# yuanzhi-zhu/DiffPIR

Measured on AMD Instinct MI355X. Metric: restored images/sec @100 NFE, 256x256, higher is better.
Workload: dtype f32 (GEMMs as 3 x f16 MFMA on hi/lo-split fp32 operands, fp32 accumulate; exact-fp32-MFMA mode in alt_precision); 1 GPU; configs[1]: ffhq topology 256x256 deblur (61x61 Gaussian PSF), 100 NFE, batch 16/GPU, device Philox noise, hipGraph=on; global_batch=16, nfe=100, collective=none

## Files before the change

### diffpir_amd/_lib.py

```python
from __future__ import annotations

import ctypes as C
import os

_HERE = os.path.dirname(os.path.abspath(__file__))
LIB_PATH = os.environ.get("DIFFPIR_LIB") or os.path.join(_HERE, "csrc", "libdiffpir_hip.so")
ABI_VERSION = 2



class UNetDesc(C.Structure):
    _fields_ = [("image_size", C.c_int32), ("in_channels", C.c_int32), ("model_channels", C.c_int32),
                ("out_channels", C.c_int32), ("num_res_blocks", C.c_int32), ("num_head_channels", C.c_int32),
                ("n_channel_mult", C.c_int32), ("channel_mult", C.c_float * 8),
                ("n_attention_ds", C.c_int32), ("attention_ds", C.c_int32 * 8), ("num_classes", C.c_int32)]


class Tensor(C.Structure):
    _fields_ = [("name", C.c_char_p), ("data", C.c_void_p), ("ndim", C.c_int32), ("shape", C.c_int64 * 4)]


class Step(C.Structure):
    _fields_ = [("t", C.c_int32), ("last", C.c_int32), ("c1", C.c_float), ("c2", C.c_float), ("tau", C.c_float),
                ("sa_t", C.c_float), ("s1m_t", C.c_float), ("sa_p", C.c_float),
# ... 9 lines not shown
                ("seed", C.c_uint64), ("image_offset", C.c_int64), ("use_graph", C.c_int32),
                ("skip_dead_final_eval", C.c_int32), ("generate_mode", C.c_int32), ("first_order", C.c_int32),
                ("noise_rp_dev", C.c_void_p), ("ddim_sample", C.c_int32)]


class InpaintRow(C.Structure):
    _fields_ = [("t", C.c_int32), ("last", C.c_int32), ("pos", C.c_int32), ("back", C.c_int32),
                ("c1", C.c_float), ("c2", C.c_float), ("tau", C.c_float), ("sa_t", C.c_float), ("s1m_t", C.c_float), ("sa_p", C.c_float),
                ("k1", C.c_float), ("q", C.c_float), ("es", C.c_float), ("k2", C.c_float),
                ("sae", C.c_float), ("sb", C.c_float), ("sa_n", C.c_float), ("s1m_n", C.c_float),
                ("mix_next", C.c_int32), ("reserved", C.c_int32)]


class DpsCoef(C.Structure):
    _fields_ = [("pc1", C.c_float), ("pc2", C.c_float), ("min_log", C.c_float), ("max_log", C.c_float), ("sa_prev", C.c_float), ("s1m_prev", C.c_float)]


class PSampleCoef(C.Structure):
    _fields_ = [("c1", C.c_float), ("c2", C.c_float), ("pc1", C.c_float), ("pc2", C.c_float), ("min_log", C.c_float), ("max_log", C.c_float),
                ("ddim", C.c_int32), ("sa_prev", C.c_float), ("s1m_prev", C.c_float)]


class DegradeDesc(C.Structure):
    _fields_ = [("task", C.c_int32), ("B", C.c_int32), ("H", C.c_int32), ("W", C.c_int32), ("sf", C.c_int32),
                ("kh", C.c_int32), ("kw", C.c_int32), ("noise_level_img", C.c_float), ("seed", C.c_uint64), ("image_offset", C.c_int64)]


class Conv3Desc(C.Structure):
    _fields_ = ([(n, C.c_int32) for n in ("B", "ca", "cb", "Cout", "H", "W", "mode", "res_mode", "scaled", "prologue", "route", "split",
                                          "defer", "Cout2")] +
                [(n, C.c_void_p) for n in ("xa", "xb", "w", "bias", "res", "prm", "gamma", "beta", "film", "gamma2", "beta2", "w2", "bias2",
                                           "out", "stat_out", "out2")] +
                [(n, C.c_int32) for n in ("stat_kind_out", "path_out", "ksplit_out", "reserved")])


PROF_CLASSES = 8
PROF_NAMES = ["conv3x3", "conv1x1", "groupnorm_stats", "attention", "fft_prox", "elementwise", "unet_forward", "loop_graph"]

SIGNATURES = {
    "dpir_version": (C.c_int, []),
    "dpir_device_count": (C.c_int, [C.POINTER(C.c_int)]),
    "dpir_create": (C.c_int, [C.c_int, C.POINTER(C.c_void_p)]),
    "dpir_destroy": (None, [C.c_void_p]),
    "dpir_last_error": (C.c_char_p, [C.c_void_p]),
    "dpir_sync": (C.c_int, [C.c_void_p]),
    "dpir_stream": (C.c_void_p, [C.c_void_p]),
    "dpir_malloc": (C.c_int, [C.c_void_p, C.c_size_t, C.POINTER(C.c_void_p)]),
    "dpir_free": (C.c_int, [C.c_void_p, C.c_void_p]),
    "dpir_h2d": (C.c_int, [C.c_void_p, C.c_void_p, C.c_void_p, C.c_size_t]),
    "dpir_d2h": (C.c_int, [C.c_void_p, C.c_void_p, C.c_void_p, C.c_size_t]),
    "dpir_d2d": (C.c_int, [C.c_void_p, C.c_void_p, C.c_void_p, C.c_size_t]),
    "dpir_load_unet": (C.c_int, [C.c_void_p, C.POINTER(UNetDesc), C.POINTER(Tensor), C.c_int]),
    "dpir_set_precision": (C.c_int, [C.c_void_p, C.c_int]),
    "dpir_unet_forward": (C.c_int, [C.c_void_p, C.c_void_p, C.c_void_p, C.c_void_p, C.c_void_p, C.c_int, C.c_int, C.c_int]),
    "dpir_model_fn_xstart": (C.c_int, [C.c_void_p, C.c_void_p, C.c_int, C.c_float, C.c_float, C.c_void_p, C.c_void_p,
                                       C.c_int, C.c_int, C.c_int]),
    "dpir_enable_grad": (C.c_int, [C.c_void_p, C.c_int]),
    "dpir_unet_vjp": (C.c_int, [C.c_void_p, C.c_void_p, C.c_void_p, C.c_void_p, C.c_void_p, C.c_void_p, C.c_void_p, C.c_int, C.c_int, C.c_int]),
    "dpir_run_dps_loop": (C.c_int, [C.c_void_p, C.POINTER(LoopDesc), C.POINTER(Step), C.POINTER(DpsCoef), C.c_int, C.c_int, C.c_float,
                                    C.c_void_p, C.c_void_p, C.c_float, C.c_void_p, C.c_void_p]),
    "dpir_p_sample": (C.c_int, [C.c_void_p, C.c_void_p, C.c_int, C.POINTER(PSampleCoef), C.c_void_p, C.c_void_p, C.c_void_p, C.c_void_p, C.c_int, C.c_int, C.c_int]),
    "dpir_eps_from_xstart": (C.c_int, [C.c_void_p, C.c_void_p, C.c_void_p, C.c_float, C.c_float, C.c_int, C.c_void_p, C.c_size_t]),
    "dpir_grad_and_value": (C.c_int, [C.c_void_p, C.c_int, C.c_void_p, C.c_void_p, C.c_int, C.c_void_p, C.c_void_p, C.c_int, C.c_int, C.c_int]),
    "dpir_blur_reflect": (C.c_int, [C.c_void_p, C.c_void_p, C.c_void_p, C.c_int, C.c_int, C.c_float, C.c_float, C.c_void_p, C.c_int, C.c_int, C.c_int]),
    "dpir_blur_reflect_adjoint": (C.c_int, [C.c_void_p, C.c_void_p, C.c_void_p, C.c_int, C.c_int, C.c_float, C.c_void_p, C.c_int, C.c_int, C.c_int]),
    "dpir_grad_and_value_blur": (C.c_int, [C.c_void_p, C.c_int, C.c_void_p, C.c_void_p, C.c_void_p, C.c_int, C.c_int, C.c_void_p, C.c_void_p,
# ... 41 lines not shown
}

_lib = None


class EngineLibraryError(RuntimeError):
    pass


DEBUG_LIB_PATH = os.path.join(_HERE, "csrc", "libdiffpir_dbg.so")
_dbg = None


def load_debug():
    global _dbg
    if _dbg is not None:
        return _dbg
    load()
    if not os.path.exists(DEBUG_LIB_PATH):
        raise EngineLibraryError(f"{DEBUG_LIB_PATH} not found: `make -C diffpir_amd/csrc` builds it next to the product library")
    d = C.CDLL(DEBUG_LIB_PATH)
    d.dpir_debug_conv_bench.argtypes = [C.c_void_p] + [C.c_int] * 10 + [C.POINTER(C.c_double)]
    d.dpir_debug_conv7_emit_supported.argtypes = [C.c_void_p] + [C.c_int] * 4 + [C.POINTER(C.c_int)]
    d.dpir_debug_victim.argtypes = [C.c_void_p, C.c_int, C.c_int, C.c_int, C.c_longlong, C.c_int, C.POINTER(C.c_ulonglong)]
    d.dpir_debug_victim_alu.argtypes = [C.c_void_p, C.c_int, C.c_int, C.c_int, C.c_int, C.POINTER(C.c_ulonglong)]
    for fn in (d.dpir_debug_victim_fft_pk, d.dpir_debug_victim_fft_nopk):
        fn.argtypes = [C.c_void_p, C.c_int, C.c_int, C.c_int, C.POINTER(C.c_ulonglong)]
    d.dpir_debug_conv7_check.argtypes = [C.c_void_p] + [C.c_int] * 10 + [C.POINTER(C.c_double), C.POINTER(C.c_double), C.POINTER(C.c_ulonglong),
                                                                        C.POINTER(C.c_float), C.POINTER(C.c_int)]
    d.dpir_debug_conv5_layer.argtypes = [C.c_void_p] + [C.c_int] * 7 + [C.c_void_p] * 7 + [C.POINTER(C.c_int)]
    d.dpir_debug_conv5_layer.restype = C.c_int
    d.dpir_debug_conv3_layer.argtypes = [C.c_void_p, C.POINTER(Conv3Desc)]
    d.dpir_debug_conv3_layer.restype = C.c_int
    for n in ("dpir_debug_conv_bench", "dpir_debug_victim", "dpir_debug_victim_alu", "dpir_debug_victim_fft_pk", "dpir_debug_victim_fft_nopk",
              "dpir_debug_conv7_check"):
        getattr(d, n).restype = C.c_int
    _dbg = d
    return d


def load():
    global _lib
    if _lib is not None:
        return _lib
    if not os.path.exists(LIB_PATH):
        raise EngineLibraryError(
            f"{LIB_PATH} not found: build it with `python -c 'import __graft_entry__ as g; g.build()'` "
            f"or `make -C diffpir_amd/csrc`.  There is no CPU fallback.")
    try:
        import torch
    except ImportError:
        pass
    try:
        lib = C.CDLL(LIB_PATH)
    except OSError as ex:
        raise EngineLibraryError(f"cannot load {LIB_PATH}: {ex}") from ex
    for name, (res, args) in SIGNATURES.items():
        try:
            fn = getattr(lib, name)
        except AttributeError as ex:
            raise EngineLibraryError(f"{LIB_PATH} does not export {name}") from ex
        fn.restype = res
        fn.argtypes = args
    if lib.dpir_version() != ABI_VERSION:
        raise EngineLibraryError("ABI version mismatch")
    _lib = lib
# ... 2 lines not shown
```

### diffpir_amd/csrc/dbg_conv.hip

```cpp
#include "engine.h"
#include "conv6_params.h"
#include "../../include/diffpir_debug.h"
#include <string.h>
#include <vector>
using namespace dpir;
static int fail(dpir_engine* e, const Status& s) {
    if (e) e->last_error = s.msg;
    return s.code;
}
#define API_TRY(e, expr)                          \
    do {                                          \
        Status _s = (expr);                       \
        if (!_s.ok()) return fail((e), _s);       \
    } while (0)
#define API_HIP(e, expr)                                                                  \
    do {                                                                                  \
        hipError_t _h = (expr);                                                           \
        if (_h != hipSuccess)                                                             \
            return fail((e), Status{DPIR_ERR_HIP, std::string(#expr) + ": " + hipGetErrorString(_h)}); \
    } while (0)

__global__ void dbg_bitdiff_kernel(const float* a, const float* b, size_t n, unsigned long long* out) {
    unsigned long long cnt = 0; unsigned mx = 0;
    for (size_t i = (size_t)blockIdx.x * blockDim.x + threadIdx.x; i < n; i += (size_t)gridDim.x * blockDim.x) {
        const float x = a[i], y = b[i];
        if (__builtin_bit_cast(unsigned, x) != __builtin_bit_cast(unsigned, y)) {
            ++cnt;
            const float d = fabsf(x - y);
            const unsigned u = d == d ? __builtin_bit_cast(unsigned, d) : 0x7fc00000u;
            mx = u > mx ? u : mx;
        }
    }
    if (cnt) { atomicAdd(&out[0], cnt); atomicMax(&out[1], (unsigned long long)mx); }
}
// ... 424 lines not shown
        ga.silu = true; ga.mode = 0; ga.B = B; ga.Hs = H; ga.Ws = W;
        ga.hi = s16b; ga.lo = x1 ? nullptr : s16b + plane2; ga.range_ctr = e->range_ctr;
        API_TRY(e, launch_gn_act_small(e->stream, ga));
        std::vector<uint16_t> w16b;
        const float w16b_scale = pack_weights_conv6(d->w2, Co2, Cn, w16b);
        void* wp2 = nullptr;
        API_TRY(e, e->ws.get("c3#w16b", w16b.size() * 2, &wp2));
        API_HIP(e, hipMemcpy(wp2, w16b.data(), w16b.size() * 2, hipMemcpyHostToDevice));
        Conv6Args c6;
        c6.x1 = x1; c6.xhi = s16b; c6.xlo = s16b + plane2; c6.w16 = wp2; c6.w16_scale = w16b_scale;
        c6.bias = dbias2; c6.out = dout2; c6.B = B; c6.Cin = Cn; c6.Cout = Co2; c6.H = H; c6.W = W;
        API_TRY(e, launch_conv6(e->stream, c6));
        API_HIP(e, hipStreamSynchronize(e->stream));
        API_HIP(e, hipMemcpy(d->out2, dout2, no2 * 4, hipMemcpyDeviceToHost));
    }
    API_HIP(e, hipStreamSynchronize(e->stream));
    API_HIP(e, hipMemcpy(d->out, dout, no * 4, hipMemcpyDeviceToHost));
    if (d->stat_out && (kind == 1 || kind == 2)) {
        if (kind == 1) {
            std::vector<float2> hs(nst);
            API_HIP(e, hipMemcpy(hs.data(), st, nst * 8, hipMemcpyDeviceToHost));
            for (size_t pl = 0; pl < (size_t)B * Cout; ++pl) {
                double s1 = 0.0, s2 = 0.0;
                for (int k = 0; k < slots; ++k) { s1 += (double)hs[pl * slots + k].x; s2 += (double)hs[pl * slots + k].y; }
                d->stat_out[2 * pl] = s1; d->stat_out[2 * pl + 1] = s2;
            }
        } else {
            API_HIP(e, hipMemcpy(d->stat_out, sp, (size_t)B * Cout * 16, hipMemcpyDeviceToHost));
        }
    }
    return DPIR_OK;
}

int dpir_debug_conv7_emit_supported(dpir_engine* e, int B, int Cout, int H, int W, int* capacity_out) {
    if (!e) return 0;
    (void)hipSetDevice(e->device);
    if (capacity_out) *capacity_out = conv7_emit_capacity();
    return conv7_emit_supported(B, Cout, H, W) ? 1 : 0;
}

}
```

### diffpir_amd/csrc/unet.hip

```cpp
#include "engine.h"
#include "conv6_params.h"
#include <unordered_map>
#include <cstdint>
#include <math.h>
#include <string.h>
#include <stdlib.h>

namespace dpir {

Status Workspace::get(const std::string& name, size_t bytes, void** out) {
    auto it = bufs.find(name);
    if (it != bufs.end() && it->second.bytes >= bytes) { *out = it->second.p; return Status{}; }
    if (frozen) return Status{DPIR_ERR_STATE, "workspace allocation of '" + name + "' during graph capture"};
    if (it != bufs.end()) { (void)hipFree(it->second.p); total -= it->second.bytes; bufs.erase(it); }
    void* p = nullptr;
    size_t rb = (bytes + 255) & ~(size_t)255;
    hipError_t err = hipMalloc(&p, rb);
    if (err != hipSuccess) return Status{DPIR_ERR_NOMEM, "hipMalloc(" + std::to_string(rb) + ") for '" + name + "' failed"};
    bufs[name] = DevBuf{p, rb};
    total += rb;
    ++generation;
    *out = p;
    return Status{};
}
void Workspace::release() {
    for (auto& kv : bufs) (void)hipFree(kv.second.p);
    bufs.clear();
    total = 0;
}

namespace {
struct WeightMap {
    std::map<std::string, const dpir_tensor*> m;
    Status find(const std::string& key, std::vector<int64_t> shape, const float** out) const {
// ... 288 lines not shown
            if (is_pending(res)) return invalid("gn_conv: residual is an unfinished convolution");
            const int C8 = 2 * ((C + 15) / 16);
            const size_t plane = (size_t)B * C8 * Ho * Wo * 16;
            char* s16 = nullptr;
            DPIR_TRY(ws.getT("act#s16", 2 * plane, &s16));
            GnActArgs ga;
            ga.src = CatSrc{in.a, in.ca, in.b, in.cb};
            ga.pend = pending;
            ga.gamma = g.gamma; ga.beta = g.beta;
            ga.film = film_off >= 0 ? film : nullptr; ga.film_stride = film_stride; ga.film_off = film_off < 0 ? 0 : film_off;
            ga.fstep = fstep; ga.frows = film_rows;
            ga.silu = true; ga.mode = mode; ga.B = B; ga.Hs = in.H; ga.Ws = in.W;
            ga.hi = s16; ga.lo = x1 ? nullptr : s16 + plane; ga.range_ctr = e->range_ctr;
            if (grad) {
                DPIR_TRY(ws.getT(tag + "#prm", (size_t)B * C, &ga.prm_out));
                DPIR_TRY(ws.getT(tag + "#gst", (size_t)B * 32, &ga.stats_out));
                if (prm_out) *prm_out = ga.prm_out;
                if (stats_out) *stats_out = ga.stats_out;
            }
            {
                ProfScope ps(&e->prof, PC_ELEM);
                DPIR_TRY(launch_gn_act_small(s, ga));
            }
            if (pending.partial) { fused.erase(pending.out); pending = PendingConv{}; }
            return conv6_on_planes(cw, s16, plane, res, res_mode, out, Ho, Wo, emit);
        }
        DPIR_TRY(resolve());
        float4* prm = nullptr;
        DPIR_TRY(gn(g, in, tag, film_off, true, &prm, stats_out));
        if (prm_out) *prm_out = prm;
        return conv(cw, in, mode, prm, res, res_mode, out, Ho, Wo, emit);
    }

    Status conv6_on_planes(const ConvW& cw, char* s16, size_t plane, const float* res, int res_mode, float* out, int Ho, int Wo,
                           const Conv6Emit* emit = nullptr) {
        const bool x1 = e->precision == 2;
        Conv6Args a6;
        a6.x1 = x1;
        a6.xhi = s16; a6.xlo = s16 + plane; a6.w16 = cw.w16; a6.w16_scale = cw.w16_scale;
        a6.bias = cw.bias; a6.out = out; a6.res = res; a6.res_mode = res_mode;
        a6.B = B; a6.Cin = cw.cin; a6.Cout = cw.cout; a6.H = Ho; a6.W = Wo;
        a6.partial = partial; a6.partial_capacity = partial_cap;
        const int slots = conv6_stat_slots(Ho, Wo);
        float2* st = nullptr; double2* sp = nullptr;
        if (slots > 0 && cw.cout % 32 == 0) {
            const std::string key = std::to_string(reinterpret_cast<uintptr_t>(out));
            DPIR_TRY(ws.getT("st#" + key, (size_t)B * cw.cout * slots, &st));
            DPIR_TRY(ws.getT("sp#" + key, (size_t)B * cw.cout, &sp));
        }
        a6.stat = st; a6.stat_plane = sp;
        a6.emit = emit;
        if (emit) { a6.stat = nullptr; a6.stat_plane = nullptr; a6.partial = nullptr; a6.partial_capacity = 0; }
        int kind = 0;
        PendingConv pc;
        ProfScope ps(&e->prof, PC_CONV3);
        DPIR_TRY(launch_conv6(s, a6, &kind, fuse_small ? &pc : nullptr));
        if (kind == 1) fused[out] = FusedStat{st, slots, nullptr};
        else if (kind == 2) fused[out] = FusedStat{nullptr, 0, sp};
        else fused.erase(out);
        if (kind == 3) pending = pc;
        return Status{};
    }

    Status conv(const ConvW& cw, const Act& in, int mode, const float4* prm, const float* res, int res_mode, float* out, int Ho, int Wo,
                const Conv6Emit* emit = nullptr) {
        const bool x1 = e->precision == 2;
        const bool use5 = cw.w16 && cw.ks == 1 && mode == 0 && (!res || res_mode == 0) && !(prm && in.C() % 16) &&
                          (conv5_supported(B, cw.cout, Ho, Wo, prm != nullptr) ||
                           conv5_small_supported(B, in.ca, in.b ? in.cb : 0, cw.cout, Ho, Wo, prm != nullptr));
        if (pending.partial && (is_pending(in.a) || is_pending(in.b) || is_pending(res) || !use5)) DPIR_TRY(resolve());
        static const bool use_conv8 = !(getenv("DPIR_CONV8") && atoi(getenv("DPIR_CONV8")) == 0);
        if (use_conv8 && cw.w8 && prm && !grad && !emit && !res && mode == 0 && !in.b && in.H == Ho && in.W == Wo &&
            conv8_supported(B, in.C(), cw.cout, Ho, Wo)) {
            Conv8Args a8;
            a8.x = in.a; a8.prm = prm; a8.w = cw.w8; a8.w_scale = cw.w8_scale; a8.bias = cw.bias; a8.out = out;
            a8.B = B; a8.C = in.C(); a8.Cout = cw.cout; a8.H = Ho; a8.W = Wo; a8.range_ctr = e->range_ctr; a8.x1 = x1;
            fused.erase(out);
            ProfScope ps(&e->prof, PC_CONV3);
            return launch_conv8(s, a8);
        }
        if (cw.w16 && cw.ks == 3 && conv6_supported(Ho, Wo)) {
            int eh = mode == 1 ? Ho / 2 : (mode == 2 ? Ho * 2 : Ho), ew = mode == 1 ? Wo / 2 : (mode == 2 ? Wo * 2 : Wo);
            if (eh != in.H || ew != in.W) return invalid("conv: source resolution does not match mode");
            const int C = in.C(), C8 = 2 * ((C + 15) / 16);
            const size_t plane = (size_t)B * C8 * Ho * Wo * 16;
            if (plane >= ((size_t)1 << 32)) return invalid("conv: split activation plane exceeds the 4 GiB buffer-descriptor range; reduce the batch");
            char* s16 = nullptr;
            DPIR_TRY(ws.getT("act#s16", 2 * plane, &s16));
// ... 112 lines not shown
            a5.bias = r.skip.bias; a5.out = sk; a5.res = nullptr; a5.B = B; a5.Cout = r.cout; a5.H = Ho; a5.W = Wo;
            a5.range_ctr = e->range_ctr; a5.x1 = x1;
            a5.emit_prm = prm1; a5.emit_hi = s16; a5.emit_lo = x1 ? nullptr : s16 + eplane;
            fused.erase(sk);
            {
                ProfScope ps(&e->prof, PC_CONV1);
                DPIR_TRY(launch_conv5(s, a5));
            }
            float* o = nullptr;
            DPIR_TRY(ws.getT(r.name + "#out", on, &o));
            if (h1_fusable(r, Ho, Wo)) {
                Conv6Emit em; char* s16b = nullptr; size_t plane2 = 0;
                DPIR_TRY(make_emit(r, Ho, Wo, &em, &s16b, &plane2));
                DPIR_TRY(conv6_on_planes(r.conv1, s16, eplane, nullptr, 0, nullptr, Ho, Wo, &em));
                DPIR_TRY(conv6_on_planes(r.conv2, s16b, plane2, sk, 0, o, Ho, Wo));
            } else {
                DPIR_TRY(conv6_on_planes(r.conv1, s16, eplane, nullptr, 0, h1, Ho, Wo));
                tap(r.name + "#h1", h1, on);
                DPIR_TRY(gn_conv(r.gn2, r.name + "#gn2", r.film_off, r.conv2, h1a, 0, sk, 0, o, Ho, Wo, &tr.prm2, &tr.st2));
            }
            tap(r.name, o, on);
            if (grad) {
                tr.idx = (int)(&r - e->net.res.data());
                tr.in = CatSrc{in.a, in.ca, in.b, in.cb}; tr.inH = in.H; tr.inW = in.W; tr.Ho = Ho; tr.Wo = Wo; tr.h1 = h1; tr.sk = sk; tr.out = o;
                e->tape.nodes.push_back(TapeNode{1, (int)e->tape.res.size()});
                e->tape.res.push_back(tr);
            }
            out->a = o; out->ca = r.cout; out->b = nullptr; out->cb = 0; out->H = Ho; out->W = Wo;
            return Status{};
        }
        TapeRes tr{};
        float* sk = nullptr;
        if (r.has_skip) DPIR_TRY(ws.getT(r.name + "#skip", on, &sk));
        const bool fuse = h1_fusable(r, Ho, Wo);
        Conv6Emit em; char* s16b = nullptr; size_t plane2 = 0;
        if (fuse) DPIR_TRY(make_emit(r, Ho, Wo, &em, &s16b, &plane2));
        DPIR_TRY(gn_conv(r.gn1, r.name + "#gn1", -1, r.conv1, in, r.mode, nullptr, 0, fuse ? nullptr : h1, Ho, Wo, &tr.prm1, &tr.st1, fuse ? &em : nullptr));
        if (!fuse) tap(r.name + "#h1", h1, on);
        if (r.has_skip) {
            DPIR_TRY(conv(r.skip, in, 0, nullptr, nullptr, 0, sk, Ho, Wo));
            res = sk;
            tr.sk = sk;
        } else {
            if (in.b) return invalid("resblock " + r.name + ": identity skip on a concatenated input");
            res = in.a; res_mode = r.mode;
        }
        float* o = nullptr;
        DPIR_TRY(ws.getT(r.name + "#out", on, &o));
        if (fuse) DPIR_TRY(conv6_on_planes(r.conv2, s16b, plane2, res, res_mode, o, Ho, Wo));
        else DPIR_TRY(gn_conv(r.gn2, r.name + "#gn2", r.film_off, r.conv2, h1a, 0, res, res_mode, o, Ho, Wo, &tr.prm2, &tr.st2));
        tap(r.name, o, on);
        if (grad) {
            tr.idx = (int)(&r - e->net.res.data());
            tr.in = CatSrc{in.a, in.ca, in.b, in.cb}; tr.inH = in.H; tr.inW = in.W; tr.Ho = Ho; tr.Wo = Wo; tr.h1 = h1; tr.out = o;
            e->tape.nodes.push_back(TapeNode{1, (int)e->tape.res.size()});
            e->tape.res.push_back(tr);
        }
        out->a = o; out->ca = r.cout; out->b = nullptr; out->cb = 0; out->H = Ho; out->W = Wo;
        return Status{};
    }

    Status attention(const AttnW& aw, const Act& in, Act* out) {
        if (in.b || in.ca != aw.c) return invalid("attention " + aw.name + ": bad input");
        int T = in.H * in.W;
        float4* prm = nullptr;
        float2* gst = nullptr;
        DPIR_TRY(resolve());
        DPIR_TRY(gn(aw.norm, in, aw.name + "#norm", -1, false, &prm, &gst));
        float *qkv = nullptr, *att = nullptr, *o = nullptr;
// ... 173 lines not shown
```

### include/diffpir_debug.h

```cpp
#ifndef DIFFPIR_DEBUG_H
#define DIFFPIR_DEBUG_H
#include "diffpir_engine.h"
#ifdef __cplusplus
extern "C" {
#endif
int dpir_debug_conv_bench(dpir_engine* e, int B, int Cin, int Cout, int H, int W, int ks, int mode, int with_prm,
                          int dbg, int iters, double* ms_out);
int dpir_debug_victim(dpir_engine* e, int lds_bytes, int threads, int blocks, long long spin_ticks, int iters, unsigned long long* bad_out);
int dpir_debug_victim_alu(dpir_engine* e, int mode, int blocks, int iters_in_kernel, int launches, unsigned long long* bad_out);
int dpir_debug_victim_fft_pk(dpir_engine* e, int blocks, int iters_in_kernel, int launches, unsigned long long* bad_out);
int dpir_debug_victim_fft_nopk(dpir_engine* e, int blocks, int iters_in_kernel, int launches, unsigned long long* bad_out);
int dpir_debug_conv7_check(dpir_engine* e, int B, int Cin, int Cout, int H, int W, int res_mode, int x1, int split, int scaled, int iters,
                           double* ms6_out, double* ms7_out, unsigned long long* mismatches_out, float* maxdiff_out, int* ksplit_out);
int dpir_debug_conv7_emit_supported(dpir_engine* e, int B, int Cout, int H, int W, int* capacity_out);
int dpir_debug_conv5_layer(dpir_engine* e, int B, int ca, int cb, int Cout, int H, int W, int tile, const float* xa, const float* xb,
                           const float* w, const float* bias, const float* prm, const float* res, float* out, int* path_out);
typedef struct dpir_debug_conv3_desc {
    int32_t B, ca, cb, Cout, H, W, mode, res_mode, scaled, prologue, route, split, defer, Cout2;
    const float *xa, *xb, *w, *bias, *res, *prm, *gamma, *beta, *film, *gamma2, *beta2, *w2, *bias2;
    float* out; double* stat_out; float* out2;
    int32_t stat_kind_out, path_out, ksplit_out, reserved;
} dpir_debug_conv3_desc;
int dpir_debug_conv3_layer(dpir_engine* e, dpir_debug_conv3_desc* d);
#ifdef __cplusplus
}
#endif
#endif
```

Measured before the change: 8.779 images/s.

## Add whole-image conv9 kernel for 8x8 layers with fused GroupNorm-SiLU emission

```diff
diff --git a/diffpir_amd/_lib.py b/diffpir_amd/_lib.py
--- a/diffpir_amd/_lib.py
+++ b/diffpir_amd/_lib.py
@@ -65,6 +65,12 @@
                 [(n, C.c_void_p) for n in ("xa", "xb", "w", "bias", "res", "prm", "gamma", "beta", "film", "gamma2", "beta2", "w2", "bias2",
                                            "out", "stat_out", "out2")] +
                 [(n, C.c_int32) for n in ("stat_kind_out", "path_out", "ksplit_out", "reserved")])
+
+
+class Conv9Desc(C.Structure):
+    _fields_ = ([(n, C.c_int32) for n in ("B", "Cin", "Cout", "H", "W", "res_mode", "hop", "Cout2")] +
+                [(n, C.c_void_p) for n in ("x", "w", "bias", "res", "prm", "gamma2", "beta2", "film2", "w2", "bias2", "out", "stat_out", "out2")] +
+                [(n, C.c_int32) for n in ("ran_out", "iters")] + [("ms_out", C.c_double)])
 
 
 PROF_CLASSES = 8
@@ -172,6 +178,8 @@
     d.dpir_debug_conv5_layer.restype = C.c_int
     d.dpir_debug_conv3_layer.argtypes = [C.c_void_p, C.POINTER(Conv3Desc)]
     d.dpir_debug_conv3_layer.restype = C.c_int
+    d.dpir_debug_conv9_layer.argtypes = [C.c_void_p, C.POINTER(Conv9Desc)]
+    d.dpir_debug_conv9_layer.restype = C.c_int
     for n in ("dpir_debug_conv_bench", "dpir_debug_victim", "dpir_debug_victim_alu", "dpir_debug_victim_fft_pk", "dpir_debug_victim_fft_nopk",
               "dpir_debug_conv7_check"):
         getattr(d, n).restype = C.c_int
diff --git a/diffpir_amd/csrc/conv9.h b/diffpir_amd/csrc/conv9.h
--- /dev/null
+++ b/diffpir_amd/csrc/conv9.h
@@ -0,0 +1,30 @@
+#pragma once
+#include "common.h"
+#include "conv6_params.h"
+namespace dpir {
+
+struct Conv9Args {
+    const void* xhi = nullptr; const void* xlo = nullptr;
+    const void* w16 = nullptr; float w16_scale = 1.f;
+    const float* bias = nullptr; float* out = nullptr; const float* res = nullptr; int res_mode = 0;
+    int B = 0, Cin = 0, Cout = 0, H = 0, W = 0;
+    double2* stat_plane = nullptr;
+    bool x1 = false;
+    const Conv6Emit* emit = nullptr;
+};
+
+struct Conv9K {
+    const char* xhi; const char* xlo; int C8;
+    const char* w16; const float* bias; float* out; const float* res; int res_mode;
+    int B, Cout, n_chunks, n_co_blocks;
+    float out_scale;
+    double2* stat;
+    Conv6Emit em;
+};
+
+constexpr int kConv9MinWg = 128;
+
+bool conv9_supported(int B, int Cin, int Cout, int H, int W, bool emit);
+Status launch_conv9(hipStream_t s, const Conv9Args& a);
+
+}
diff --git a/diffpir_amd/csrc/conv9.hip b/diffpir_amd/csrc/conv9.hip
--- /dev/null
+++ b/diffpir_amd/csrc/conv9.hip
@@ -0,0 +1,321 @@
+#include "common.h"
+#include "elem.h"
+#include "lds_dma.h"
+#include "conv9.h"
+#include <type_traits>
+
+namespace dpir {
+
+typedef float floatx16 __attribute__((ext_vector_type(16)));
+typedef _Float16 half8 __attribute__((ext_vector_type(8)));
+
+template <int I, int N, class F>
+__device__ __forceinline__ void static_for9(F&& f) {
+    if constexpr (I < N) {
+        f(std::integral_constant<int, I>{});
+        static_for9<I + 1, N>(f);
+    }
+}
+
+__device__ __forceinline__ float silu9(float v) {
+    float e = __builtin_amdgcn_exp2f(v * -1.4426950408889634f);
+    return v * __builtin_amdgcn_rcpf(1.0f + e);
+}
+
+constexpr int kC9WaveLds = 16384;
+constexpr int kC9RedStride = 68;
+constexpr int kC9RedBytes = 4 * 32 * kC9RedStride * 4;
+constexpr int kC9Lds = 4 * kC9WaveLds;
+static_assert(kC9RedBytes + 512 + 2 * 4096 <= kC9Lds, "epilogue areas");
+
+template <int HW, bool X1, bool EMIT>
+__global__ __launch_bounds__(256, 1) void conv9_image_kernel(Conv9K p) {
+#if defined(__HIP_DEVICE_COMPILE__)
+    static_assert(HW == 64, "the 8 x 8 image is the one built");
+    constexpr int W = 8, H = 8, LW = W + 2, LH = H + 2;
+    constexpr int PATCH = LH * LW;
+    constexpr int NPIECE = (2 * PATCH + 63) / 64;
+    constexpr int XB = NPIECE * 1024;
+    constexpr int NPL = X1 ? 1 : 2;
+    constexpr int NACT = NPL * NPIECE;
+    constexpr int TAPS = 9;
+    static_assert(2 * 2 * XB == kC9WaveLds, "per-wave staging");
+    extern __shared__ __attribute__((aligned(16))) char smem9[];
+
+    const int tid = threadIdx.x;
+    const int lane = tid & 63;
+    const int wave = __builtin_amdgcn_readfirstlane(tid >> 6);
+    const int l31 = lane & 31;
+    const int half = lane >> 5;
+
+    const int tiles = p.Cout >> 5;
+    const int bid = blockIdx.x;
+    int cot, n;
+    if ((tiles & 7) == 0) { cot = (bid & 7) + 8 * (bid / (8 * p.B)); n = (bid >> 3) % p.B; }
+    else { cot = bid % tiles; n = bid / tiles; }
+    const int co_blk = cot >> 2, ct = cot & 3;
+
+    unsigned x_off[NPIECE];
+#pragma unroll
+    for (int u = 0; u < NPIECE; ++u) {
+        const int f = u * 64 + lane;
+        const int kg = f / PATCH;
+        const int e = f - kg * PATCH;
+        const int hy = e / LW, hx = e - hy * LW;
+        const int gy = hy - 1, gx = hx - 1;
+        const bool ok = kg < 2 && gy >= 0 && gy < H && gx >= 0 && gx < W;
+        x_off[u] = ok ? ((unsigned)((n * p.C8 + kg) * HW + gy * W + gx) << 4) : kOutOfRange;
+    }
+    const size_t xplane_bytes = (size_t)p.B * p.C8 * HW * 16;
+    char* const wlds = smem9 + wave * kC9WaveLds;
+    auto dma_x = [&](int chunk, int buf, int q) __attribute__((always_inline)) {
+        const int u = X1 ? q : q >> 1, plane = X1 ? 0 : q & 1;
+        const size_t coff = (size_t)chunk * 2 * HW * 16;
+        const __amdgpu_buffer_rsrc_t rx = rsrc_uniform((plane ? p.xlo : p.xhi) + coff, (unsigned)(xplane_bytes - coff));
+        BLDS6(rx, wlds + buf * 2 * XB + plane * XB + u * 1024, x_off[u], 0);
+    };
+
+    const int lane_b = (l31 >> 3) * LW + (l31 & 7) + half * PATCH;
+    const half8* xbase = reinterpret_cast<const half8*>(wlds) + lane_b;
+
+    const unsigned lane16 = (unsigned)lane * 16u;
+    half8 a_h[TAPS], a_l[TAPS];
+    auto load_a = [&](int chunk, auto tap_c) __attribute__((always_inline)) {
+        constexpr int tap = decltype(tap_c)::value;
+        const char* base = p.w16 + (((size_t)chunk * p.n_co_blocks + co_blk) * 4 + ct) * (TAPS * 2048);
+        const __amdgpu_buffer_rsrc_t rw = rsrc_uniform(base, TAPS * 2048);
+        a_h[tap] = __builtin_bit_cast(half8, __builtin_amdgcn_raw_buffer_load_b128(rw, lane16, tap * 2048u, 0));
+        if (!X1) a_l[tap] = __builtin_bit_cast(half8, __builtin_amdgcn_raw_buffer_load_b128(rw, lane16, tap * 2048u + 1024u, 0));
+    };
+
+    floatx16 acc[2];
+#pragma unroll
+    for (int j = 0; j < 2; ++j)
+#pragma unroll
+        for (int r = 0; r < 16; ++r) acc[j][r] = 0.f;
+
+    half8 b_h[3][2], b_l[3][2];
+    auto read_b = [&](int buf, auto tap_c, auto set_c) __attribute__((always_inline)) {
+        constexpr int tap = decltype(tap_c)::value, set = decltype(set_c)::value;
+        constexpr int toff = (tap / 3) * LW + (tap % 3);
+        const half8* xh = xbase + buf * (2 * XB / 16);
+        const half8* xl = xh + XB / 16;
+#pragma unroll
+        for (int j = 0; j < 2; ++j) {
+            b_h[set][j] = xh[j * 4 * LW + toff];
+            if (!X1) b_l[set][j] = xl[j * 4 * LW + toff];
+        }
+    };
+
+    auto chunk_body = [&](auto more_c, int chunk, int cur) __attribute__((always_inline)) {
+        constexpr bool MORE = decltype(more_c)::value;
+        if (MORE) {
+#pragma unroll
+            for (int q = 0; q < NACT; ++q) dma_x(chunk + 4, cur ^ 1, q);
+        }
+        static_for9<0, TAPS>([&](auto tap_c) __attribute__((always_inline)) {
+            constexpr int tap = decltype(tap_c)::value;
+            constexpr int set = tap == 0 ? 2 : (tap & 1);
+            __builtin_amdgcn_sched_barrier(0);
+            if constexpr (tap + 1 < TAPS) {
+                read_b(cur, std::integral_constant<int, tap + 1>{}, std::integral_constant<int, (tap + 1) & 1>{});
+            } else if (MORE) {
+                wait_vmcnt<(TAPS - 1) * NPL>();
+                barrier_lds_only();
+                read_b(cur ^ 1, std::integral_constant<int, 0>{}, std::integral_constant<int, 2>{});
+            }
+            __builtin_amdgcn_sched_barrier(0);
+            if (!X1) {
+#pragma unroll
+                for (int j = 0; j < 2; ++j) acc[j] = __builtin_amdgcn_mfma_f32_32x32x16_f16(a_l[tap], b_h[set][j], acc[j], 0, 0, 0);
+#pragma unroll
+                for (int j = 0; j < 2; ++j) acc[j] = __builtin_amdgcn_mfma_f32_32x32x16_f16(a_h[tap], b_l[set][j], acc[j], 0, 0, 0);
+            }
+#pragma unroll
+            for (int j = 0; j < 2; ++j) acc[j] = __builtin_amdgcn_mfma_f32_32x32x16_f16(a_h[tap], b_h[set][j], acc[j], 0, 0, 0);
+            __builtin_amdgcn_sched_barrier(0);
+            if (MORE) load_a(chunk + 4, tap_c);
+        });
+        __builtin_amdgcn_sched_barrier(0);
+    };
+
+    const int rounds = (p.n_chunks + 3) >> 2;
+    int chunk = wave;
+    if (chunk < p.n_chunks) {
+#pragma unroll
+        for (int q = 0; q < NACT; ++q) dma_x(chunk, 0, q);
+        static_for9<0, TAPS>([&](auto tap_c) __attribute__((always_inline)) { load_a(chunk, tap_c); });
+    }
+    wait_vmcnt<0>();
+    __syncthreads();
+    if (chunk < p.n_chunks) read_b(0, std::integral_constant<int, 0>{}, std::integral_constant<int, 2>{});
+    for (int it = 0; it < rounds; ++it, chunk += 4) {
+        if (chunk + 4 < p.n_chunks) {
+            chunk_body(std::true_type{}, chunk, it & 1);
+        } else {
+            if (chunk < p.n_chunks) chunk_body(std::false_type{}, chunk, it & 1);
+            barrier_lds_only();
+        }
+    }
+
+    float* const red = reinterpret_cast<float*>(smem9);
+#pragma unroll
+    for (int j = 0; j < 2; ++j)
+#pragma unroll
+        for (int r = 0; r < 16; ++r)
+            red[(wave * 32 + (r & 3) + 8 * (r >> 2) + 4 * half) * kC9RedStride + j * 32 + l31] = acc[j][r];
+    __syncthreads();
+    const int ch = tid >> 3, seg = tid & 7;
+    const int co = cot * 32 + ch;
+    float v[8];
+#pragma unroll
+    for (int w = 0; w < 4; ++w) {
+        const float4 lo4 = *reinterpret_cast<const float4*>(red + (w * 32 + ch) * kC9RedStride + seg * 8);
+        const float4 hi4 = *reinterpret_cast<const float4*>(red + (w * 32 + ch) * kC9RedStride + seg * 8 + 4);
+        const float t[8] = {lo4.x, lo4.y, lo4.z, lo4.w, hi4.x, hi4.y, hi4.z, hi4.w};
+#pragma unroll
+        for (int i = 0; i < 8; ++i) v[i] = w == 0 ? t[i] : v[i] + t[i];
+    }
+    {
+        const float osc = p.out_scale, bv = p.bias[co];
+#pragma unroll
+        for (int i = 0; i < 8; ++i) v[i] = v[i] * osc + bv;
+    }
+    const size_t plane = (size_t)n * p.Cout + co;
+
+    if constexpr (!EMIT) {
+        if (p.res) {
+            float r[8];
+            if (p.res_mode == 0) {
+                const float4 a = *reinterpret_cast<const float4*>(p.res + plane * HW + seg * 8), b = *reinterpret_cast<const float4*>(p.res + plane * HW + seg * 8 + 4);
+                r[0] = a.x; r[1] = a.y; r[2] = a.z; r[3] = a.w; r[4] = b.x; r[5] = b.y; r[6] = b.z; r[7] = b.w;
+            } else if (p.res_mode == 1) {
+                const float4 a = *reinterpret_cast<const float4*>(p.res + plane * (HW / 4) + (seg >> 1) * (W / 2));
+                r[0] = a.x; r[1] = a.x; r[2] = a.y; r[3] = a.y; r[4] = a.z; r[5] = a.z; r[6] = a.w; r[7] = a.w;
+            } else {
+                const float* rp = p.res + plane * (4 * HW) + (size_t)(2 * seg) * (2 * W);
+#pragma unroll
+                for (int h4 = 0; h4 < 4; ++h4) {
+                    const float4 a = *reinterpret_cast<const float4*>(rp + h4 * 4), b = *reinterpret_cast<const float4*>(rp + 2 * W + h4 * 4);
+                    r[2 * h4] = ((a.x + a.y) + (b.x + b.y)) * 0.25f;
+                    r[2 * h4 + 1] = ((a.z + a.w) + (b.z + b.w)) * 0.25f;
+                }
+            }
+#pragma unroll
+            for (int i = 0; i < 8; ++i) v[i] = r[i] + v[i];
+        }
+        float* op = p.out + plane * HW + seg * 8;
+        *reinterpret_cast<float4*>(op) = make_float4(v[0], v[1], v[2], v[3]);
+        *reinterpret_cast<float4*>(op + 4) = make_float4(v[4], v[5], v[6], v[7]);
+        if (p.stat) {
+            double s = (((double)v[0] + (double)v[1]) + ((double)v[2] + (double)v[3])) + (((double)v[4] + (double)v[5]) + ((double)v[6] + (double)v[7]));
+            double ss = (((double)v[0] * v[0] + (double)v[1] * v[1]) + ((double)v[2] * v[2] + (double)v[3] * v[3])) +
+                        (((double)v[4] * v[4] + (double)v[5] * v[5]) + ((double)v[6] * v[6] + (double)v[7] * v[7]));
+#pragma unroll
+            for (int o = 4; o > 0; o >>= 1) { s += __shfl_xor(s, o, 64); ss += __shfl_xor(ss, o, 64); }
+            if (seg == 0) p.stat[plane] = make_double2(s, ss);
+        }
+    } else {
+        double2* const chs = reinterpret_cast<double2*>(smem9 + kC9RedBytes);
+        _Float16* const th = reinterpret_cast<_Float16*>(smem9 + kC9RedBytes + 512);
+        {
+            double s = 0.0, ss = 0.0;
+#pragma unroll
+            for (int i = 0; i < 8; ++i) { s += (double)v[i]; ss += (double)v[i] * v[i]; }
+#pragma unroll
+            for (int o = 4; o > 0; o >>= 1) { s += __shfl_xor(s, o, 64); ss += __shfl_xor(ss, o, 64); }
+            if (seg == 0) chs[ch] = make_double2(s, ss);
+        }
+        __syncthreads();
+        const int cg = p.Cout >> 5;
+        const int g0 = (ch / cg) * cg;
+        double S = 0.0, SS = 0.0;
+        for (int k = 0; k < cg; ++k) { S += chs[g0 + k].x; SS += chs[g0 + k].y; }
+        const double cntd = (double)cg * HW;
+        const double mean = S / cntd;
+        double var = SS / cntd - mean * mean;
+        if (var < 0) var = 0;
+        const float rstd = (float)(1.0 / sqrt(var + 1e-5));
+        float a = rstd * p.em.gamma[co];
+        float b = p.em.beta[co];
+        if (p.em.film) {
+            const float* f = p.em.film + (p.em.fstep ? (size_t)p.em.fstep->i * p.em.frows : 0) + (size_t)n * p.em.film_stride + p.em.film_off;
+            const float sc = 1.0f + f[co];
+            const float sh = f[p.Cout + co];
+            a = a * sc;
+            b = b * sc + sh;
+        }
+        const float meanf = (float)mean;
+        bool bad = false;
+#pragma unroll
+        for (int i = 0; i < 8; ++i) {
+            float x = (v[i] - meanf) * a + b;
+            x = silu9(x);
+            bad |= !(fabsf(x) <= 65000.f);
+            x = fminf(fmaxf(x, -65000.f), 65000.f);
+            const _Float16 h = (_Float16)x;
+            th[(seg * 8 + i) * 32 + ch] = h;
+            if (!X1) th[2048 + (seg * 8 + i) * 32 + ch] = (_Float16)(x - (float)h);
+        }
+        __syncthreads();
+        {
+            typedef unsigned int u32x4e __attribute__((ext_vector_type(4)));
+            const int c8l = tid >> 6, px = tid & 63;
+            const size_t eo = (((size_t)n * p.em.C8 + (cot * 4 + c8l)) * HW + px) << 4;
+            *reinterpret_cast<u32x4e*>(p.em.hi + eo) = *reinterpret_cast<const u32x4e*>(th + px * 32 + c8l * 8);
+            if (!X1) *reinterpret_cast<u32x4e*>(p.em.lo + eo) = *reinterpret_cast<const u32x4e*>(th + 2048 + px * 32 + c8l * 8);
+        }
+        const unsigned long long mk = __ballot(bad);
+        if (mk != 0ull && lane == (int)__builtin_ctzll(mk)) atomicAdd(p.em.range_ctr, (unsigned long long)__builtin_popcountll(mk));
+    }
+#endif
+}
+
+template <bool X1, bool EMIT>
+static Status launch9(hipStream_t s, const Conv9K& k, int blocks) {
+    auto fn = conv9_image_kernel<64, X1, EMIT>;
+    static LdsAttrOnce attr_set;
+    DPIR_HIP(attr_set.set(reinterpret_cast<const void*>(fn), kC9Lds));
+    hipLaunchKernelGGL(fn, dim3((unsigned)blocks), dim3(256), kC9Lds, s, k);
+    return Status{};
+}
+
+static const char* conv9_refusal(int B, int Cin, int Cout, int H, int W, bool emit) {
+    if (B <= 0 || Cin <= 0 || Cout <= 0) return "conv9: empty launch";
+    if (H != W) return "conv9: whole-image tiles need a square image";
+    if (H != 8) return "conv9: the whole-image tile is built for 8 x 8 layers only";
+    if (Cin % 16) return "conv9: the input channels must be a multiple of 16";
+    if (Cout % 32) return "conv9: the output channels must be a multiple of 32";
+    if (emit && 32 % (Cout / 32) != 0) return "conv9: fused emission needs GroupNorm groups that do not straddle a 32-channel tile";
+    if ((size_t)B * (Cin / 8) * H * W * 16 >= ((size_t)1 << 32)) return "conv9: split activation plane exceeds the 4 GiB buffer-descriptor range";
+    return nullptr;
+}
+
+bool conv9_supported(int B, int Cin, int Cout, int H, int W, bool emit) { return conv9_refusal(B, Cin, Cout, H, W, emit) == nullptr; }
+
+Status launch_conv9(hipStream_t s, const Conv9Args& a) {
+    const bool emit = a.emit != nullptr;
+    if (const char* why = conv9_refusal(a.B, a.Cin, a.Cout, a.H, a.W, emit)) return Status{DPIR_ERR_UNSUPPORTED, why};
+    if (!a.xhi || (!a.x1 && !a.xlo) || !a.w16 || !a.bias) return invalid("conv9: operand planes, f16 weight pack and bias are required");
+    if (a.res && (a.res_mode < 0 || a.res_mode > 2)) return invalid("conv9: bad residual mode");
+    Conv9K k{};
+    k.xhi = reinterpret_cast<const char*>(a.xhi); k.xlo = reinterpret_cast<const char*>(a.xlo); k.C8 = a.Cin / 8;
+    k.w16 = reinterpret_cast<const char*>(a.w16); k.bias = a.bias; k.out = a.out; k.res = a.res; k.res_mode = a.res_mode;
+    k.B = a.B; k.Cout = a.Cout; k.n_chunks = a.Cin / 16; k.n_co_blocks = (a.Cout + 127) / 128;
+    k.out_scale = 1.0f / a.w16_scale;
+    k.stat = a.stat_plane;
+    const int blocks = a.B * (a.Cout / 32);
+    if (emit) {
+        if (a.res || !a.emit->hi || (!a.x1 && !a.emit->lo) || !a.emit->gamma || !a.emit->beta || !a.emit->range_ctr || a.emit->C8 != a.Cout / 8)
+            return invalid("conv9: fused emission takes no residual and needs the next convolution's planes, gamma, beta and the range guard");
+        k.em = *a.emit;
+        DPIR_TRY(a.x1 ? (launch9<true, true>(s, k, blocks)) : (launch9<false, true>(s, k, blocks)));
+    } else {
+        if (!a.out) return invalid("conv9: no output");
+        DPIR_TRY(a.x1 ? (launch9<true, false>(s, k, blocks)) : (launch9<false, false>(s, k, blocks)));
+    }
+    DPIR_HIP(hipGetLastError());
+    return Status{};
+}
+
+}
diff --git a/diffpir_amd/csrc/dbg_conv.hip b/diffpir_amd/csrc/dbg_conv.hip
--- a/diffpir_amd/csrc/dbg_conv.hip
+++ b/diffpir_amd/csrc/dbg_conv.hip
@@ -1,5 +1,6 @@
 #include "engine.h"
 #include "conv6_params.h"
+#include "conv9.h"
 #include "../../include/diffpir_debug.h"
 #include <string.h>
 #include <vector>
@@ -490,6 +491,110 @@
     return DPIR_OK;
 }
 
+int dpir_debug_conv9_layer(dpir_engine* e, dpir_debug_conv9_desc* d) {
+    if (!e || !d) return DPIR_ERR_INVALID;
+    d->ran_out = 0;
+    const int B = d->B, Cin = d->Cin, Cout = d->Cout, H = d->H, W = d->W;
+    if (!d->x || !d->w || !d->bias || B <= 0 || Cin <= 0 || Cout <= 0 || H <= 0 || W <= 0 || d->res_mode < -1 || d->res_mode > 2 ||
+        (d->res_mode >= 0 && !d->res) || (!d->hop && !d->out) || (d->hop && (!d->gamma2 || !d->beta2 || !d->w2 || !d->bias2 || !d->out2 || d->Cout2 <= 0)))
+        return fail(e, invalid("conv9 layer: bad descriptor"));
+    if (e->grad_enabled) return fail(e, Status{DPIR_ERR_UNSUPPORTED, "conv9 layer: a gradient-mode engine keeps launch_conv6's route"});
+    if (e->precision == 0) return fail(e, Status{DPIR_ERR_UNSUPPORTED, "conv9 layer: the f32 precision keeps the fp32 kernel"});
+    if (d->hop && d->res_mode >= 0) return fail(e, invalid("conv9 layer: the hop's first layer takes no residual"));
+    if ((d->res_mode == 1 && ((H | W) & 1))) return fail(e, invalid("conv9 layer: a half-resolution residual needs an even output size"));
+    (void)hipSetDevice(e->device);
+    const bool x1 = e->precision == 2;
+    const size_t HW = (size_t)H * W, nx = (size_t)B * Cin * HW, no = (size_t)B * Cout * HW;
+    const size_t nres = d->res_mode == 1 ? no / 4 : (d->res_mode == 2 ? no * 4 : no);
+    const int chunks = (Cin + 15) / 16, C8 = 2 * chunks;
+    const size_t plane = (size_t)B * C8 * HW * 16;
+    float *dx = nullptr, *dbias = nullptr, *dout = nullptr, *dres = nullptr; float4* dprm = nullptr; double2* sp = nullptr; char* s16 = nullptr;
+    API_TRY(e, e->ws.getT("c9#x", nx, &dx));
+    API_TRY(e, e->ws.getT("c9#b", (size_t)round_up(Cout, 64), &dbias));
+    API_TRY(e, e->ws.getT("c9#o", no, &dout));
+    API_TRY(e, e->ws.getT("c9#res", nres, &dres));
+    API_TRY(e, e->ws.getT("c9#prm", (size_t)B * Cin, &dprm));
+    API_TRY(e, e->ws.getT("c9#sp", (size_t)B * Cout, &sp));
+    API_TRY(e, e->ws.getT("c9#s16", 2 * plane, &s16));
+    API_HIP(e, hipMemcpy(dx, d->x, nx * 4, hipMemcpyHostToDevice));
+    API_HIP(e, hipMemset(dbias, 0, (size_t)round_up(Cout, 64) * 4));
+    API_HIP(e, hipMemcpy(dbias, d->bias, (size_t)Cout * 4, hipMemcpyHostToDevice));
+    if (d->prm) API_HIP(e, hipMemcpy(dprm, d->prm, (size_t)B * Cin * 16, hipMemcpyHostToDevice));
+    if (d->res_mode >= 0) API_HIP(e, hipMemcpy(dres, d->res, nres * 4, hipMemcpyHostToDevice));
+    API_HIP(e, hipMemsetAsync(dout, 0xFF, no * 4, e->stream));
+    API_HIP(e, hipMemsetAsync(sp, 0xFF, (size_t)B * Cout * 16, e->stream));
+    API_HIP(e, hipMemsetAsync(s16, 0xFF, 2 * plane, e->stream));
+    API_TRY(e, launch_act_split(e->stream, CatSrc{dx, Cin, nullptr, 0}, d->prm ? dprm : nullptr, 0, B, H, W, s16, x1 ? nullptr : s16 + plane, e->range_ctr));
+    std::vector<uint16_t> w16v;
+    const float w16_scale = pack_weights_conv6(d->w, Cout, Cin, w16v);
+    void* wp = nullptr;
+    API_TRY(e, e->ws.get("c9#w16", w16v.size() * 2, &wp));
+    API_HIP(e, hipMemcpy(wp, w16v.data(), w16v.size() * 2, hipMemcpyHostToDevice));
+    Conv9Args a9;
+    a9.xhi = s16; a9.xlo = s16 + plane; a9.w16 = wp; a9.w16_scale = w16_scale; a9.bias = dbias; a9.out = dout;
+    if (d->res_mode >= 0) { a9.res = dres; a9.res_mode = d->res_mode; }
+    a9.B = B; a9.Cin = Cin; a9.Cout = Cout; a9.H = H; a9.W = W; a9.stat_plane = sp; a9.x1 = x1;
+    d->ms_out = 0.0;
+    auto timed = [&](auto&& launch) -> int {
+        if (d->iters <= 0) return DPIR_OK;
+        hipEvent_t e0, e1;
+        API_HIP(e, hipEventCreate(&e0)); API_HIP(e, hipEventCreate(&e1));
+        API_HIP(e, hipEventRecord(e0, e->stream));
+        for (int i = 0; i < d->iters; ++i) API_TRY(e, launch());
+        API_HIP(e, hipEventRecord(e1, e->stream));
+        API_HIP(e, hipEventSynchronize(e1));
+        float ms = 0; API_HIP(e, hipEventElapsedTime(&ms, e0, e1));
+        (void)hipEventDestroy(e0); (void)hipEventDestroy(e1);
+        d->ms_out = ms / d->iters;
+        return DPIR_OK;
+    };
+    if (!d->hop) {
+        API_TRY(e, launch_conv9(e->stream, a9));
+        if (int rc = timed([&]() { return launch_conv9(e->stream, a9); })) return rc;
+        API_HIP(e, hipStreamSynchronize(e->stream));
+        d->ran_out = 1;
+        API_HIP(e, hipMemcpy(d->out, dout, no * 4, hipMemcpyDeviceToHost));
+        if (d->stat_out) API_HIP(e, hipMemcpy(d->stat_out, sp, (size_t)B * Cout * 16, hipMemcpyDeviceToHost));
+        return DPIR_OK;
+    }
+    const int Co2 = d->Cout2, C8b = 2 * ((Cout + 15) / 16);
+    const size_t plane2 = (size_t)B * C8b * HW * 16, no2 = (size_t)B * Co2 * HW;
+    char* s16b = nullptr; float *dg = nullptr, *db = nullptr, *df = nullptr, *dbias2 = nullptr, *dout2 = nullptr;
+    API_TRY(e, e->ws.getT("c9#s16b", 2 * plane2, &s16b));
+    API_TRY(e, e->ws.getT("c9#gamma2", (size_t)Cout, &dg));
+    API_TRY(e, e->ws.getT("c9#beta2", (size_t)Cout, &db));
+    API_TRY(e, e->ws.getT("c9#film2", (size_t)B * 2 * Cout, &df));
+    API_TRY(e, e->ws.getT("c9#b2", (size_t)round_up(Co2, 64), &dbias2));
+    API_TRY(e, e->ws.getT("c9#o2", no2, &dout2));
+    API_HIP(e, hipMemsetAsync(s16b, 0xFF, 2 * plane2, e->stream));
+    API_HIP(e, hipMemcpy(dg, d->gamma2, (size_t)Cout * 4, hipMemcpyHostToDevice));
+    API_HIP(e, hipMemcpy(db, d->beta2, (size_t)Cout * 4, hipMemcpyHostToDevice));
+    if (d->film2) API_HIP(e, hipMemcpy(df, d->film2, (size_t)B * 2 * Cout * 4, hipMemcpyHostToDevice));
+    API_HIP(e, hipMemset(dbias2, 0, (size_t)round_up(Co2, 64) * 4));
+    API_HIP(e, hipMemcpy(dbias2, d->bias2, (size_t)Co2 * 4, hipMemcpyHostToDevice));
+    API_HIP(e, hipMemsetAsync(dout2, 0xFF, no2 * 4, e->stream));
+    std::vector<uint16_t> w16b;
+    const float w16b_scale = pack_weights_conv6(d->w2, Co2, Cout, w16b);
+    void* wp2 = nullptr;
+    API_TRY(e, e->ws.get("c9#w16b", w16b.size() * 2, &wp2));
+    API_HIP(e, hipMemcpy(wp2, w16b.data(), w16b.size() * 2, hipMemcpyHostToDevice));
+    Conv6Emit em;
+    em.hi = s16b; em.lo = x1 ? nullptr : s16b + plane2; em.C8 = C8b; em.gamma = dg; em.beta = db;
+    em.film = d->film2 ? df : nullptr; em.film_stride = 2 * Cout; em.film_off = 0; em.frows = 2 * Cout; em.fstep = nullptr;
+    em.range_ctr = e->range_ctr;
+    a9.out = nullptr; a9.stat_plane = nullptr; a9.emit = &em;
+    API_TRY(e, launch_conv9(e->stream, a9));
+    Conv9Args b9;
+    b9.xhi = s16b; b9.xlo = s16b + plane2; b9.w16 = wp2; b9.w16_scale = w16b_scale; b9.bias = dbias2; b9.out = dout2;
+    b9.B = B; b9.Cin = Cout; b9.Cout = Co2; b9.H = H; b9.W = W; b9.x1 = x1;
+    API_TRY(e, launch_conv9(e->stream, b9));
+    if (int rc = timed([&]() -> Status { DPIR_TRY(launch_conv9(e->stream, a9)); return launch_conv9(e->stream, b9); })) return rc;
+    API_HIP(e, hipStreamSynchronize(e->stream));
+    d->ran_out = 1;
+    API_HIP(e, hipMemcpy(d->out2, dout2, no2 * 4, hipMemcpyDeviceToHost));
+    return DPIR_OK;
+}
+
 int dpir_debug_conv7_emit_supported(dpir_engine* e, int B, int Cout, int H, int W, int* capacity_out) {
     if (!e) return 0;
     (void)hipSetDevice(e->device);
diff --git a/diffpir_amd/csrc/unet.hip b/diffpir_amd/csrc/unet.hip
--- a/diffpir_amd/csrc/unet.hip
+++ b/diffpir_amd/csrc/unet.hip
@@ -1,5 +1,6 @@
 #include "engine.h"
 #include "conv6_params.h"
+#include "conv9.h"
 #include <unordered_map>
 #include <cstdint>
 #include <math.h>
@@ -354,6 +355,13 @@
         return conv(cw, in, mode, prm, res, res_mode, out, Ho, Wo, emit);
     }
 
+    bool conv9_route(const ConvW& cw, int Ho, int Wo, bool hop) const {
+        static const bool on = !(getenv("DPIR_CONV9") && atoi(getenv("DPIR_CONV9")) == 0);
+        static const int min_wg = getenv("DPIR_CONV9_MIN_WG") ? atoi(getenv("DPIR_CONV9_MIN_WG")) : kConv9MinWg;
+        return on && !grad && e->precision != 0 && cw.w16 && cw.ks == 3 && conv9_supported(B, cw.cin, cw.cout, Ho, Wo, hop) &&
+               (long long)B * (cw.cout / 32) >= min_wg;
+    }
+
     Status conv6_on_planes(const ConvW& cw, char* s16, size_t plane, const float* res, int res_mode, float* out, int Ho, int Wo,
                            const Conv6Emit* emit = nullptr) {
         const bool x1 = e->precision == 2;
@@ -376,6 +384,16 @@
         int kind = 0;
         PendingConv pc;
         ProfScope ps(&e->prof, PC_CONV3);
+        if (conv9_route(cw, Ho, Wo, emit != nullptr)) {
+            Conv9Args a9;
+            a9.xhi = s16; a9.xlo = s16 + plane; a9.w16 = cw.w16; a9.w16_scale = cw.w16_scale; a9.bias = cw.bias; a9.out = out;
+            a9.res = res; a9.res_mode = res_mode; a9.B = B; a9.Cin = cw.cin; a9.Cout = cw.cout; a9.H = Ho; a9.W = Wo;
+            a9.stat_plane = emit ? nullptr : sp; a9.x1 = x1; a9.emit = emit;
+            DPIR_TRY(launch_conv9(s, a9));
+            if (sp && !emit) fused[out] = FusedStat{nullptr, 0, sp};
+            else fused.erase(out);
+            return Status{};
+        }
         DPIR_TRY(launch_conv6(s, a6, &kind, fuse_small ? &pc : nullptr));
         if (kind == 1) fused[out] = FusedStat{st, slots, nullptr};
         else if (kind == 2) fused[out] = FusedStat{nullptr, 0, sp};
@@ -554,9 +572,18 @@
         TapeRes tr{};
         float* sk = nullptr;
         if (r.has_skip) DPIR_TRY(ws.getT(r.name + "#skip", on, &sk));
-        const bool fuse = h1_fusable(r, Ho, Wo);
+        const bool hop9 = fuse_h1 && !grad && r.gn2.c == r.cout && conv9_route(r.conv1, Ho, Wo, true) && conv9_route(r.conv2, Ho, Wo, false);
+        const bool fuse = hop9 || h1_fusable(r, Ho, Wo);
         Conv6Emit em; char* s16b = nullptr; size_t plane2 = 0;
-        if (fuse) DPIR_TRY(make_emit(r, Ho, Wo, &em, &s16b, &plane2));
+        if (hop9) {
+            const int C8 = r.cout / 8;
+            plane2 = (size_t)B * C8 * Ho * Wo * 16;
+            DPIR_TRY(ws.getT("act#s16b", 2 * plane2, &s16b));
+            em.hi = s16b; em.lo = e->precision == 2 ? nullptr : s16b + plane2; em.C8 = C8;
+            em.gamma = r.gn2.gamma; em.beta = r.gn2.beta;
+            em.film = r.film_off >= 0 ? film : nullptr; em.film_stride = film_stride; em.film_off = r.film_off < 0 ? 0 : r.film_off;
+            em.frows = film_rows; em.fstep = fstep; em.range_ctr = e->range_ctr;
+        } else if (fuse) DPIR_TRY(make_emit(r, Ho, Wo, &em, &s16b, &plane2));
         DPIR_TRY(gn_conv(r.gn1, r.name + "#gn1", -1, r.conv1, in, r.mode, nullptr, 0, fuse ? nullptr : h1, Ho, Wo, &tr.prm1, &tr.st1, fuse ? &em : nullptr));
         if (!fuse) tap(r.name + "#h1", h1, on);
         if (r.has_skip) {
diff --git a/include/diffpir_debug.h b/include/diffpir_debug.h
--- a/include/diffpir_debug.h
+++ b/include/diffpir_debug.h
@@ -22,6 +22,14 @@
     int32_t stat_kind_out, path_out, ksplit_out, reserved;
 } dpir_debug_conv3_desc;
 int dpir_debug_conv3_layer(dpir_engine* e, dpir_debug_conv3_desc* d);
+typedef struct dpir_debug_conv9_desc {
+    int32_t B, Cin, Cout, H, W, res_mode, hop, Cout2;
+    const float *x, *w, *bias, *res, *prm, *gamma2, *beta2, *film2, *w2, *bias2;
+    float* out; double* stat_out; float* out2;
+    int32_t ran_out, iters;
+    double ms_out;
+} dpir_debug_conv9_desc;
+int dpir_debug_conv9_layer(dpir_engine* e, dpir_debug_conv9_desc* d);
 #ifdef __cplusplus
 }
 #endif
```

Result: faster. 8.874 images/s, median of 6 (+1.1%).
